# kangxiongbin/HyLight

Measured on AMD Instinct MI355X. Metric: long-read all-vs-all overlaps/sec, higher is better.
Workload: dtype u8/int32

## Files before the change

### hylight_amd/csrc/ava_align.hip

```cpp
#include <algorithm>
#include <memory>
#include <type_traits>

#include "ava_internal.h"
#include "dev_prims.h"
#include "wave_ops.h"

namespace hlmi {

namespace {
constexpr int WG = 256;
constexpr int WAVES = WG / 64;
constexpr int SEQ_T_MAX = EXT_MAX + BAND_W;
constexpr int NR_SHORT = 128;
constexpr int WIDE_SHORT = 128;
inline dim3 grid1(size_t n) { return grid_for(n, WG); }

struct Task {
    uint32_t piece;
    uint16_t kind;
    uint16_t narrow;
    uint64_t qa, ta;
    int16_t m, n;
    int16_t dlo;
    int16_t trim;
};
constexpr uint16_t TASK_REV = 4;
constexpr uint16_t TASK_ONE = 8;
struct TaskOut {
    int32_t score;
    int32_t bi, bj;
    uint32_t runs_off, n_runs;
    uint32_t pad;
// ... 148 lines not shown
    return off;
}

__device__ __forceinline__ uint32_t load_codes4(const uint8_t *base, long long idx, long long total) {
    if (idx >= 0 && idx + 4 <= total) {
        uint32_t v;
        __builtin_memcpy(&v, base + idx, 4);
        return v;
    }
    uint32_t v = 0;
    for (int k = 0; k < 4; ++k) v |= (uint32_t)(idx + k >= 0 && idx + k < total ? base[idx + k] : 4) << (8 * k);
    return v;
}
__device__ __forceinline__ uint32_t comp_codes4(uint32_t x) {
    const uint32_t n = x & 0x04040404u;
    return (x ^ 0x03030303u) & ~((n >> 1) | (n >> 2));
}
__device__ __forceinline__ uint32_t load_window4(const uint8_t *codes, long long total, long long a0, bool down, bool comp, int x) {
    uint32_t v = down ? __builtin_bswap32(load_codes4(codes, a0 - x - 3, total)) : load_codes4(codes, a0 + x, total);
    if (comp) v = comp_codes4(v);
    return v;
}

__device__ __forceinline__ uint32_t load_window4p(const uint8_t *codes, long long a0, bool down, bool comp, int x) {
    uint32_t v;
    __builtin_memcpy(&v, codes + (down ? a0 - x - 3 : a0 + x), 4);
    if (down) v = __builtin_bswap32(v);
    if (comp) v = comp_codes4(v);
    return v;
}


enum { ST_BASES = 0, ST_BASES_SQUARE, ST_BASES_NARROW, ST_BASES_WIDE, ST_FAST, ST_DP, ST_DP_ROWS, ST_NARROW_SMALL, ST_WIDE_ONE, ST_STUB_EXT, ST_EXT_CERT, ST_EXT_DP_ROW, ST_EXT_DP_K, ST_LONG, ST_BASES_LONG, ST_PACKED, N_ALIGN_STATS };
constexpr int NR_SMALL = 64;
constexpr uint8_t CLS_LONG = 5;
constexpr uint8_t CLS_LONG32 = 7;
constexpr uint8_t CLS_UNGAPPED = 6;

__device__ __forceinline__ uint64_t load_codes8(const uint8_t *base, long long idx, long long total) {
    if (idx >= 0 && idx + 8 <= total) {
        uint64_t v;
        __builtin_memcpy(&v, base + idx, 8);
        return v;
    }
    uint64_t v = 0;
    for (int k = 0; k < 8; ++k) v |= (uint64_t)(idx + k >= 0 && idx + k < total ? base[idx + k] : 4) << (8 * k);
    return v;
}
__device__ __forceinline__ uint64_t load_window8(const uint8_t *codes, long long total, long long a0, bool down, bool comp, int x) {
    uint64_t v = down ? __builtin_bswap64(load_codes8(codes, a0 - x - 7, total)) : load_codes8(codes, a0 + x, total);
    if (comp) {
        const uint64_t n = v & 0x0404040404040404ull;
        v = (v ^ 0x0303030303030303ull) & ~((n >> 1) | (n >> 2));
    }
    return v;
}

__device__ __forceinline__ uint64_t load_window8p(const uint8_t *codes, long long a0, bool down, bool comp, int x) {
    uint64_t v;
    __builtin_memcpy(&v, codes + (down ? a0 - x - 7 : a0 + x), 8);
    if (down) v = __builtin_bswap64(v);
    if (comp) {
        const uint64_t n = v & 0x0404040404040404ull;
        v = (v ^ 0x0303030303030303ull) & ~((n >> 1) | (n >> 2));
    }
    return v;
// ... 19 lines not shown
        x = (x | x >> 1) & 0x33333333u;
        x = (x | x >> 2) & 0x0f0f0f0fu;
        x = (x | x >> 4) & 0x00ff00ffu;
        return (x | x >> 8) & 0xffffu;
    };
    return even((uint32_t)d) | even((uint32_t)(d >> 32)) << 16;
}
__device__ __forceinline__ uint32_t squeeze8(uint64_t f) {
    return (((uint32_t)f * 0x10204080u) >> 28) | (((uint32_t)(f >> 32) * 0x10204080u) >> 28) << 4;
}
__device__ __forceinline__ uint32_t ne_bits8(uint64_t q, uint64_t t) {
    const uint64_t d = q ^ t;
    return squeeze8((d | d >> 1 | d >> 2) & 0x0101010101010101ull);
}
__device__ __forceinline__ uint32_t amb_bits8(uint64_t q, uint64_t t) { return squeeze8((q | t) >> 2 & 0x0101010101010101ull); }
__device__ __forceinline__ bool range_flagged(const uint32_t *nflag, long long lo, long long hi) {
    const uint32_t g0 = (uint32_t)((lo + (long long)DevReads::PAD) >> 5), g1 = (uint32_t)((hi + (long long)DevReads::PAD) >> 5);
    uint32_t any = 0;
    for (uint32_t w = g0 >> 5; w <= g1 >> 5; ++w) {
        uint32_t keep = ~0u;
        if (w == g0 >> 5) keep &= ~0u << (g0 & 31);
        if (w == g1 >> 5) keep &= ~0u >> (31 - (g1 & 31));
        any |= nflag[w] & keep;
    }
    return any != 0;
}
__device__ __forceinline__ bool window_flagged(const uint32_t *nflag, long long a0, bool down, int len) {
    return down ? range_flagged(nflag, a0 - (len - 1), a0) : range_flagged(nflag, a0, a0 + (len - 1));
}

template <int PASS>
__global__ __launch_bounds__(WG) __attribute__((amdgpu_waves_per_eu(PASS == 1 ? 4 : 5))) void classify_kernel(AlignArgs a, uint8_t *cls, unsigned long long *stats) {
    __shared__ unsigned long long s_stat[WAVES][N_ALIGN_STATS];
    constexpr int CMP_WORDS = PASS == 1 ? 64 * (BLOCK_MAX / 32) : 1;
    __shared__ uint32_t s_mm[WAVES][CMP_WORDS], s_up[WAVES][CMP_WORDS], s_dn[WAVES][CMP_WORDS];
    __shared__ uint64_t s_qa[WAVES][PASS == 1 ? 64 : 1], s_ta[WAVES][PASS == 1 ? 64 : 1];
    __shared__ uint32_t s_geo[WAVES][PASS == 1 ? 64 : 1], s_amb[WAVES][2];
    const int lane = threadIdx.x & 63;
    const size_t tid = blockIdx.x * (size_t)blockDim.x + threadIdx.x;
    const size_t n_thr = (size_t)gridDim.x * blockDim.x;
    uint32_t chunk_off = 0, chunk_left = 0;
    uint32_t st[N_ALIGN_STATS] = {};
    const size_t n_units = PASS == 1 ? a.n_tasks : (size_t)*a.defer_count;
    const size_t rounds = (n_units + n_thr - 1) / n_thr;
    TaskRef ref_n{0, 0};
    uint32_t ti_n = 0;
    if (PASS == 1) { if (tid < n_units) ref_n = a.geom.ref[tid]; }
    else if (tid < n_units) ti_n = a.defer_list[tid];
    for (size_t r = 0; r < rounds; ++r) {
        const size_t u = r * n_thr + tid;
        bool live = u < n_units;
        const size_t ti = PASS == 1 || !live ? u : (size_t)ti_n;
        TaskRef ref = ref_n;
        if (PASS == 2 && live) ref = a.geom.ref[ti];
        {
            const size_t un = u + n_thr;
            if (PASS == 1) { if (un < n_units) ref_n = a.geom.ref[un]; }
            else if (un < n_units) ti_n = a.defer_list[un];
        }
        Task tk{};
        bool held = false;
        bool bare = false;
        if (live) {
            const uint32_t pc = ref.pk & 0x3fffffffu, kind = ref.pk >> 30;
            const PieceGeom pg = a.geom.pg[pc];
            held = PASS == 1 && kind != 0 && pg.stub_cand != 0;
            bare = a.cls_bare != nullptr && pg.stub_cand != 0;
            const FixPt f0 = a.geom.fps[ref.fp];
            FixPt f1{0, 0};
            if (kind == 0) f1 = a.geom.fps[ref.fp + 1];
            tk = build_task(pg, pc, kind, f0, f1, a.ext_max);
        }
        const int m = tk.m, n = tk.n;
        uint8_t c = 2;
        bool try_fast = false;
        if (live) {
            if (m <= 0 || n <= 0 || held) c = 0;
            else if ((tk.kind & 3) == 0) {
                if (m > BLOCK_MAX || n > BLOCK_MAX)
                    c = (n > m ? n - m : m - n) <= HALF_DELTA ? CLS_LONG32 : CLS_LONG;
                else { c = tk.narrow ? (m <= NR_SHORT ? 1 : 3) : 2; try_fast = (m == n); }
            } else if ((m < n - tk.dlo ? m : n - tk.dlo) > EXT_MAX) { c = CLS_LONG32; tk.dlo = (int16_t)(-(HALF_W / 2 - 1)); }
            else if (a.ext_all_long) c = CLS_LONG;
            if (c == 2 && (m < n - tk.dlo ? m : n - tk.dlo) <= WIDE_SHORT) c = 4;
        }
        if (PASS == 1 && live) {
            const bool defer = c != 0 && a.kmax >= 0 && ((tk.kind & 3) != 0 || (m != n && c != CLS_LONG && c != CLS_LONG32));
            a.defer_flag[ti] = defer ? 1 : 0;
            if (defer) { live = false; try_fast = false; }
        }
        int k = 0, mpos[3] = {0, 0, 0}, last_x = -1;
        bool ambig = false, shift_ok = false;
        if constexpr (PASS == 1) {
            const int wv = threadIdx.x >> 6;
            bool flagged = false;
            if (try_fast && a.qpacked)
                flagged = window_flagged(a.qnflag, (long long)tk.qa, (tk.kind & TASK_REV) != 0, m) || window_flagged(a.tnflag, (long long)tk.ta, false, m);
            const bool use_packed = a.qpacked != nullptr && __ballot(flagged) == 0;
            uint32_t *mm = s_mm[wv], *mup = s_up[wv], *mdn = s_dn[wv];
            const uint32_t nch = try_fast ? (uint32_t)(m + 31) >> 5 : 0u;
            const uint32_t incl = wave_prefix_sum_incl_dpp(nch), tot = (uint32_t)__builtin_amdgcn_readlane((int)incl, 63);
            const uint32_t st0 = incl - nch;
            if (lane < 2) s_amb[wv][lane] = 0;
            s_qa[wv][lane] = tk.qa; s_ta[wv][lane] = tk.ta;
            auto compare = [&](auto packed_form) {
                constexpr bool PK = decltype(packed_form)::value;
                constexpr int PB = PK ? 32 : 8, PW = 32 / PB;
                constexpr uint32_t FIRST = PK ? 3u : 0xffu;
                using piece_t = std::conditional_t<PK, uint32_t, uint8_t>;
                piece_t *own = (piece_t *)mm, *pm = (piece_t *)mm, *pup = (piece_t *)mup, *pdn = (piece_t *)mdn;
                const uint32_t ptot = tot * PW, pst0 = st0 * PW;
                auto window = [&](bool query, int o, bool rv, int x) {
                    if constexpr (PK) return query ? load_window32p(a.qpacked, (long long)s_qa[wv][o], rv, rv, x) : load_window32p(a.tpacked, (long long)s_ta[wv][o], false, false, x);
                    else return query ? load_window8p(a.qcodes, (long long)s_qa[wv][o], rv, rv, x) : load_window8p(a.tcodes, (long long)s_ta[wv][o], false, false, x);
                };
                for (uint32_t c = (uint32_t)lane; c < ptot; c += 64) own[c] = 0;
                s_geo[wv][lane] = pst0 | (uint32_t)m << 16 | ((tk.kind & TASK_REV) ? 0x80000000u : 0u);
                __builtin_amdgcn_s_waitcnt(0xc07f);
                __builtin_amdgcn_wave_barrier();
                if (nch) own[pst0] = (piece_t)lane;
                __builtin_amdgcn_s_waitcnt(0xc07f);
                __builtin_amdgcn_wave_barrier();
// ... 312 lines not shown
        if (bare) nr = 0;
        uint32_t wave_total;
        const uint32_t mine = wave_excl_sum_u32(nr, lane, wave_total);
        uint32_t base = 0;
        bool ok = true;
        if (wave_total) {
            if (lane == 0) base = pool_take(a, wave_total, chunk_off, chunk_left, ok);
            base = (uint32_t)__shfl((int)base, 0, 64);
            ok = __shfl((int)ok, 0, 64) != 0;
        }
        if (fast) {
            if (ok) for (uint32_t q = 0; q < nr; ++q) a.runs[base + mine + q] = runs[q];
            const bool ext = (tk.kind & 3) != 0;
            const int L = ext_take >= 0 ? ext_take : (m < n ? m : n);
            a.out[ti] = TaskOut{fast_score, ext ? L : m, ext ? L : n, base + mine, ok ? nr : 0, (nr ? end_codes(runs[0], runs[nr - 1]) : 0u) | ext_flag};
        } else if (live && c == 0) {
            a.out[ti] = TaskOut{0, 0, 0, 0, 0, 0};
        }
        int m_dp = m;
        if (live && !fast && (c == 1 || c == 3) && a.kmax >= 0 && last_x >= 0 && a.trim_ok && !a.ungapped) {
            const int mn = m < n ? m : n;
            int T = mn - 1 - last_x;
            T = T < mn - 1 ? T : mn - 1;
            if (T > 0) {
                tk.m = (int16_t)(m - T); tk.n = (int16_t)(n - T); tk.trim = (int16_t)T;
                m_dp = m - T;
                c = m_dp <= NR_SHORT ? 1 : 3;
            }
        }
        if (live) {
            if (a.ungapped && c != 0) c = CLS_UNGAPPED;
            cls[ti] = bare ? 0 : c;
            if (a.cls_bare) a.cls_bare[ti] = bare ? c : 0;
            if (c != 0) a.tasks[ti] = tk;
            if (held) ++st[ST_STUB_EXT];
            else if (m > 0 && n > 0) {
                const uint32_t bases = (uint32_t)(m + n);
                st[ST_BASES] += bases;
                if ((tk.kind & 3) == 0 && m == n) st[ST_BASES_SQUARE] += bases;
                if (c == 0) ++st[ST_FAST];
                else {
                    ++st[ST_DP];
                    if (c == CLS_LONG || c == CLS_LONG32) { ++st[ST_LONG]; st[ST_BASES_LONG] += bases; st[ST_DP_ROWS] += (uint32_t)(m < n - tk.dlo ? m : n - tk.dlo); }
                    else if (c == 2 || c == 4) { st[ST_BASES_WIDE] += bases; st[ST_DP_ROWS] += (uint32_t)(m < n - tk.dlo ? m : n - tk.dlo); }
                    else { st[ST_BASES_NARROW] += bases; st[ST_DP_ROWS] += (uint32_t)m_dp; if (c == 1 && m_dp < NR_SMALL && !bare) ++st[ST_NARROW_SMALL]; }
                }
            }
        }
    }
#pragma unroll
    for (int k = 0; k < N_ALIGN_STATS; ++k) {
        unsigned long long v = st[k];
#pragma unroll
        for (int o = 32; o > 0; o >>= 1) v += __shfl_xor(v, o, 64);
        if (lane == 0) s_stat[threadIdx.x >> 6][k] = v;
    }
    __syncthreads();
    if (threadIdx.x < N_ALIGN_STATS) {
        unsigned long long v = 0;
        for (int w = 0; w < WAVES; ++w) v += s_stat[w][threadIdx.x];
        if (v) atomicAdd(&stats[threadIdx.x], v);
    }
}

__global__ void task_rows_key_kernel(const Task *tasks, const uint32_t *list, size_t n, uint32_t *key) {
    size_t i = blockIdx.x * (size_t)blockDim.x + threadIdx.x;
    if (i < n) key[i] = (uint32_t)tasks[list[i]].m >> 2;
}


__global__ void task_rows_desc_key_kernel(const Task *tasks, const uint32_t *list, size_t n, uint32_t *key) {
    size_t i = blockIdx.x * (size_t)blockDim.x + threadIdx.x;
    if (i >= n) return;
    const Task &t = tasks[list[i]];
    const int rows = (int)t.m < (int)t.n - (int)t.dlo ? (int)t.m : (int)t.n - (int)t.dlo;
    key[i] = 0xffffu - (uint32_t)(rows < 0 ? 0 : rows);
}

constexpr int DP_BIAS = 1 << 24;
constexpr int NT_PAD = 16;
constexpr int NT_EXTRA = NT_PAD + NARROW_DELTA + NARROW_W + 7;
enum { PL_DIAG = 0, PL_EGEF, PL_EEXT, PL_FEXT, PL_NE, N_PLANES };

__device__ __forceinline__ uint32_t shift_in(uint32_t acc, bool bit) {
#if defined(__HIP_DEVICE_COMPILE__)
    const unsigned long long m = __ballot(bit);
    unsigned long long co;
    asm("v_addc_co_u32 %0, %1, %2, %2, %3" : "=v"(acc), "=s"(co) : "v"(acc), "s"(m));
#endif
    return acc;
}

struct NarrowWalk {
    const uint32_t *pl;
    int chunks;
// ... 1586 lines not shown
    const size_t n_waves = ((size_t)gridDim.x * blockDim.x) >> 6;
    for (size_t i = wave; i < n; i += n_waves) {
        const Piece p = pieces[i];
        const uint32_t to = off[i];
        for (uint32_t k = (uint32_t)lane; k < p.n_fp; k += 64) dst[to + k] = src[p.fp_off + k];
        if (lane == 0) pieces[i].fp_off = fp_base + to;
    }
}
}

struct PieceSpan { struct { const Piece *p; } pieces; size_t n_pieces, n_fp; struct { const FixPt *p; } fps; };
static void align_span(const AvaInput &in, const hlmi_ava_opts &o, const uint32_t *d_qlen, const uint32_t *d_tlen,
                       const PieceSpan &ch, AlignOut &out) {
    out = AlignOut();
    const size_t P = ch.n_pieces;
    if (!P) return;
    DBuf<uint32_t> tcnt(P), toff(P);
    hipLaunchKernelGGL(piece_task_count_kernel, grid1(P), dim3(WG), 0, stream(), ch.pieces.p, P, tcnt.p);
    exclusive_scan_u32(tcnt.p, toff.p, P);
    const size_t NT = ch.n_fp + P;
    DBuf<Task> tasks(NT);
    if (P >= (1u << 30)) fail(HLMI_EINVAL, "more than 2^30 alignment pieces in one batch");
    DBuf<TaskRef> task_ref(NT);
    DBuf<PieceGeom> pgeom(P);
    if (NT <= 17 * P)
        hipLaunchKernelGGL(task_ref_lane_kernel, grid1(P), dim3(WG), 0, stream(), ch.pieces.p, toff.p, P, d_qlen, d_tlen, in.Q->off.p, in.T->off.p,
                           ch.fps.p, o.stub_oh, ext_rows(o), task_ref.p, pgeom.p);
    else
    hipLaunchKernelGGL(task_ref_kernel, dim3((unsigned)std::min<size_t>(cdiv(P, (size_t)WAVES), 256 * 32)), dim3(WG), 0, stream(),
                       ch.pieces.p, toff.p, P, d_qlen, d_tlen, in.Q->off.p, in.T->off.p, ch.fps.p, o.stub_oh, ext_rows(o), task_ref.p, pgeom.p);
    HIP_CHECK(hipGetLastError());
    DBuf<TaskOut> tout(NT);
    DBuf<uint32_t> counters(2);
    DBuf<unsigned long long> astats(N_ALIGN_STATS);
    constexpr size_t MAX_BLOCKS = 256 * 16;
    const size_t open_chunks = MAX_BLOCKS * (4 * WAVES * RUN_CHUNK + 2 * 4 * WAVES * RUN_CHUNK_SMALL) +
                               (size_t)3 * 256 * 32 * 8 * PK_WAVES * RUN_CHUNK_SMALL;
    size_t run_share = std::max<size_t>(NT * 12, 1 << 16);
    DBuf<uint32_t> runs;
    AsmArgs as{};
    as.pieces = ch.pieces.p; as.fps = ch.fps.p; as.task_off = toff.p; as.tout = tout.p; as.n_pieces = P;
    as.min_dp_score = o.min_dp_score; as.end_bonus = o.end_bonus;
    as.qlen = d_qlen; as.tlen = d_tlen; as.rank_q = in.d_rank_q; as.rank_t = in.d_rank_t; as.chunk_of_t = in.d_chunk_of_t;
    as.pg = pgeom.p; as.stub_score = o.min_dp_score + std::max(0, o.end_bonus);
    as.stage_cap = (uint32_t)ASM_STAGE;
    if (const char *e = hook("HLMI_ASM_STAGE_CAP")) as.stage_cap = (uint32_t)std::min(ASM_STAGE, std::max(0, atoi(e)));
    DBuf<uint32_t> nops(P);
    DBuf<uint8_t> valid(P), late(o.stub_oh >= 0 ? P : 0);
    DBuf<uint32_t> late_idx(o.stub_oh >= 0 ? P : 0);
    size_t n_late = 0;
    const unsigned nba = (unsigned)std::min<size_t>(cdiv(P, (size_t)WAVES), 256 * 32);
    const bool small_pieces = NT <= 17 * P && !hook("HLMI_ASM_WAVE");
    const int worst = std::max(std::max(o.match, o.mismatch), std::max(o.ambi, o.gap_open + o.gap_ext));
    const bool packed = worst > 0 && (long long)worst * (BLOCK_MAX + NARROW_W + 2) <= 4000 && o.match >= 0 && o.mismatch >= 0 &&
                        o.ambi >= 0 && o.gap_open >= 0 && o.gap_ext >= 0 && !hook("HLMI_NARROW_UNPACKED");
    const bool bare = o.stub_oh >= 0 && packed && !hook("HLMI_STUB_FULL_ROWS");
    as.bare = bare ? 1 : 0;
    if (long_rows_cap(o) > 32000) fail(HLMI_EINVAL, "max_gap %d: alignment tasks are limited to 32 000 rows", o.max_gap);
    bool ext_all_long = false;
    if (o.zdrop > 0) {
        const int D = std::max(std::max(o.mismatch, o.ambi), o.gap_open + o.gap_ext);
        const int rows_down = D > 0 ? (o.zdrop + D - 1) / D : EXT_MAX;
        ext_all_long = (long long)o.match * (EXT_MAX - rows_down) + std::max(o.end_bonus, 0) > o.zdrop;
    }
    const uint32_t long_chunks_cap = (uint32_t)(long_rows_cap(o) + 31) / 32, long_runs_cap = (uint32_t)(2 * long_rows_cap(o) + 64);
    constexpr unsigned LONG_BLOCKS_MAX = 256 * 8;
    struct LongLaunch { DBuf<uint32_t> list, planes, runs, ctl; };
    std::vector<std::unique_ptr<LongLaunch>> long_launches;
    struct LongReady { AlignArgs al; LongArgs la; unsigned nb; bool half, tb; const char *timer; };
    std::vector<LongReady> long_ready;
    hipEvent_t long_done = nullptr;
    bool long_pending = false, long_on_side = false;
    struct SideGuard {
        ~SideGuard() { if (hipStream_t s = side_stream_if_created()) (void)hipStreamSynchronize(s); }
    } side_guard;
    auto join_long = [&]() {
        if (!long_pending) return;
        if (long_on_side) {
            if (!long_done) HIP_CHECK(hipEventCreateWithFlags(&long_done, hipEventDisableTiming));
            HIP_CHECK(hipEventRecord(long_done, side_stream()));
            HIP_CHECK(hipStreamWaitEvent(stream(), long_done, 0));
            long_on_side = false;
        }
        long_pending = false;
    };
    DBuf<uint8_t> long_flag;
    DBuf<uint32_t> long_list, long_n(1);
    size_t n_long_tb = 0, n_long_bare = 0;
    double long_rows_run = 0;
    static const char *const LB_NAMES[] = {"align_narrow_small", "align_narrow", "align_narrow_long", "align_wide", "align_wide_short",
                                           "align_long", "align_score_narrow", "align_score_narrow_long", "align_score_wide",
                                           "align_score_wide_short", "align_score_long", "align_ungapped", "align_long32",
                                           "align_score_long32"};
    constexpr int N_LB = 14;
    DBuf<unsigned long long> lb_bases(N_LB + 2);
    std::vector<double> lb_n(N_LB, 0.0);
    lb_bases.zero();
    auto note_list = [&](const char *timer, const Task *tk, const uint32_t *lst, size_t n) {
        if (!n) return;
        int slot = 0;
        while (slot < N_LB && strcmp(LB_NAMES[slot], timer) != 0) ++slot;
        if (slot == N_LB) return;
        lb_n[slot] += (double)n;
        (void)tk; (void)lst;
    };
    for (int attempt = 0;; ++attempt) {
        const size_t cap_runs = run_share + open_chunks;
        if (cap_runs >= (1ull << 32)) fail(HLMI_ENOMEM, "CIGAR run pool exceeds 4G entries");
        runs.alloc(cap_runs);
        counters.zero();
        lb_bases.zero();
        std::fill(lb_n.begin(), lb_n.end(), 0.0);
        AlignArgs aa{};
        aa.tasks = tasks.p; aa.n_tasks = NT;
        aa.geom = TaskGeom{task_ref.p, pgeom.p, ch.fps.p};
        aa.qcodes = in.Q->codes(); aa.tcodes = in.T->codes();
        aa.q_total = (long long)in.Q->total; aa.t_total = (long long)in.T->total;
        if (!hook("HLMI_CLASSIFY_BYTES")) {
            if (!in.Q->packed_store.p || !in.T->packed_store.p) fail(HLMI_ESTATE, "alignment of a read set without its 2-bit copy (DevReads::pack)");
            aa.qpacked = in.Q->packed(); aa.tpacked = in.T->packed();
            aa.qnflag = in.Q->nflag.p; aa.tnflag = in.T->nflag.p;
        }
        aa.end_bonus = o.end_bonus;
        aa.ext_max = ext_rows(o);
        aa.ext_all_long = ext_all_long ? 1 : 0;
        aa.ungapped = o.bandwidth == 0 ? 1 : 0;
        aa.match = o.match; aa.mismatch = o.mismatch; aa.go = o.gap_open; aa.ge = o.gap_ext; aa.ambi = o.ambi;
// ... 4 lines not shown
            const int den = o.match + o.mismatch, num = o.match + 2 * (o.gap_open + o.gap_ext);
            aa.kmax = den > 0 && num > 0 ? std::min(3, (num - 1) / den) : 0;
            if (o.match <= 0 || o.gap_open < 0 || o.gap_ext <= 0) aa.kmax = -1;
            const int k = aa.kmax + 1, U = den, T = num;
            aa.kgap1 = aa.kmax >= 0 && U < o.gap_open + 2 * o.gap_ext + o.match && !hook("HLMI_NO_GAP1_CERT") ? 1 : 0;
            {
                auto c = [&](int L) { int v = o.gap_open + o.gap_ext * L; if (o.gap_open2 > 0) v = std::min(v, o.gap_open2 + o.gap_ext2 * L); return v; };
                aa.kgap2 = aa.kgap1 && U < o.match + c(2) && 2 * U < o.match + 2 * c(1) && 2 * U < 2 * o.match + c(2) + c(3) - c(1) &&
                           c(2) == o.gap_open + 2 * o.gap_ext && c(1) == o.gap_open + o.gap_ext && !hook("HLMI_NO_GAP2_CERT") ? 1 : 0;
            }
            aa.kshift = aa.kmax >= 0 && k <= 3 && k * U > T && k * U < T + o.match + std::min(2 * o.gap_ext, o.gap_open + o.gap_ext) &&
                        !hook("HLMI_NO_SHIFT_CERT") ? 1 : 0;
        }
        aa.trim_ok = hook("HLMI_NO_SUFFIX_TRIM") ? 0 : 1;
        aa.one_ok = hook("HLMI_NO_ONE_PIECE_CERT") ? 0 : 1;
        {
            const int U = o.match + o.mismatch;
            int G = o.gap_open + o.gap_ext;
            if (aa.go2 > 0) G = std::min(G, aa.go2 + aa.ge2);
            const bool sane = aa.kmax >= 0 && o.match > 0 && o.mismatch >= 0 && !hook("HLMI_NO_EXT_CERT");
            aa.kext_plain = sane && G >= U && U < 2 * G + o.match ? 1 : 0;
            aa.kext_bonus = 0;
            for (int k = 1; k <= 2; ++k)
                if (sane && o.end_bonus > 0 && k * U < G && k * U < o.end_bonus + o.match && k * U < 2 * G + o.match) aa.kext_bonus = k;
        }
        aa.out = tout.p; aa.runs = runs.p; aa.cap_runs = (uint32_t)cap_runs; aa.counters = counters.p;
        as.runs = runs.p;
        aa.run_buf_cap = 0xffffffffu;
        if (const char *e = hook("HLMI_RUN_BUF_CAP")) aa.run_buf_cap = (uint32_t)std::max(0, atoi(e));
        DBuf<uint8_t> cls(NT), f1(NT), cls_bare(bare ? NT : 0);
        DBuf<uint32_t> list1(NT), list2(NT), list3(NT), list4(NT);
        DBuf<uint32_t> list_n(4);
        aa.cls_bare = bare ? cls_bare.p : nullptr;
        auto class_list = [&](const uint8_t *cls_arr, uint8_t v) -> size_t {
            if (long_flag.n < NT) { long_flag.alloc(NT); long_list.alloc(NT); }
            hipLaunchKernelGGL(class_flag_kernel, grid1(NT), dim3(WG), 0, stream(), cls_arr, NT, v, long_flag.p);
            select_flagged_indices_async(long_flag.p, long_list.p, NT, long_n.p);
            return (size_t)long_n.download(1)[0];
        };
        auto run_ungapped = [&](const uint8_t *cls_arr, bool tb) -> size_t {
            if (!aa.ungapped) return 0;
            const size_t nl = class_list(cls_arr, CLS_UNGAPPED);
            if (!nl) return 0;
            aa.list = long_list.p; aa.n_list = nl;
            note_list("align_ungapped", tasks.p, long_list.p, nl);
            KTimer kt("align_ungapped");
            const unsigned nb = (unsigned)std::min<size_t>(cdiv(nl, (size_t)WG), MAX_BLOCKS);
            if (tb) hipLaunchKernelGGL(align_ungapped_kernel<true>, dim3(nb), dim3(WG), 0, stream(), aa, o.zdrop);
            else hipLaunchKernelGGL(align_ungapped_kernel<false>, dim3(nb), dim3(WG), 0, stream(), aa, o.zdrop);
            HIP_CHECK(hipGetLastError());
            return nl;
        };
        auto run_long_class = [&](const uint8_t *cls_arr, bool tb, uint8_t cv) -> size_t {
            const bool half = cv == CLS_LONG32;
            const char *timer = half ? (tb ? "align_long32" : "align_score_long32") : (tb ? "align_long" : "align_score_long");
            const size_t nl = class_list(cls_arr, cv);
            if (!nl) return 0;
            note_list(timer, tasks.p, long_list.p, nl);
            hipLaunchKernelGGL(list_ext_kernel, dim3((unsigned)std::min<size_t>(cdiv(nl, (size_t)WG), 1024)), dim3(WG), 0, stream(), tasks.p,
                               long_list.p, nl, lb_bases.p + N_LB);
            long_launches.emplace_back(new LongLaunch());
            LongLaunch &L = *long_launches.back();
            {
                DBuf<uint32_t> key(nl);
                hipLaunchKernelGGL(task_rows_desc_key_kernel, grid1(nl), dim3(WG), 0, stream(), tasks.p, long_list.p, nl, key.p);
                L.list.alloc(nl);
                HIP_CHECK(hipMemcpyAsync(L.list.p, long_list.p, nl * 4, hipMemcpyDeviceToDevice, stream()));
                sort_pairs_u32_u32(key, L.list, nl, 0, 16);
            }
            const size_t units = half ? (nl + 1) / 2 : nl;
            const unsigned nb = (unsigned)std::min<size_t>((units + WAVES - 1) / WAVES, LONG_BLOCKS_MAX);
// ... 28 lines not shown
                } else {
                    if (r.tb) { if (two) go(align_long_kernel<true, true>); else go(align_long_kernel<false, true>); }
                    else { if (two) go(align_long_kernel<true, false>); else go(align_long_kernel<false, false>); }
                }
            }
            HIP_CHECK(hipGetLastError());
            long_ready.clear();
            long_pending = true;
        };
        auto run_long = [&](const uint8_t *cls_arr, bool tb) -> size_t {
            if (aa.ungapped) return run_ungapped(cls_arr, tb);
            const size_t n32 = run_long_class(cls_arr, tb, CLS_LONG32);
            return n32 + run_long_class(cls_arr, tb, CLS_LONG);
        };
        auto check_long = [&]() {
            for (auto &L : long_launches) {
                if (!L->ctl.n) continue;
                const std::vector<uint32_t> c = L->ctl.download(4);
                if (c[1]) fail(HLMI_EINVAL, "an alignment task exceeds the scratch area of align_long_kernel");
                long_rows_run += (double)((unsigned long long)c[3] << 32 | c[2]);
                L->ctl.release(); L->planes.release(); L->runs.release(); L->list.release();
            }
        };
        size_t n_bare_tasks = 0;
        auto run_bare_long = [&]() {
            if (!bare) return;
            const size_t nl = run_long(cls_bare.p, false);
            n_bare_tasks += nl; n_long_bare += nl;
        };
        auto run_bare = [&](bool with_long) {
            if (!bare) return;
            if (with_long) { run_bare_long(); launch_long_ready(); }
            select_classes4_async(cls_bare.p, NT, list1.p, list2.p, list3.p, list4.p, list_n.p);
            const std::vector<uint32_t> hb = list_n.download(4);
            n_bare_tasks += (size_t)hb[0] + hb[1] + hb[2] + hb[3];
            for (int which = 0; which < 2; ++which) {
                DBuf<uint32_t> &lst = which ? list3 : list1;
                const size_t nl = which ? hb[2] : hb[0];
                if (nl < 8) continue;
                DBuf<uint32_t> key(nl);
                hipLaunchKernelGGL(task_rows_key_kernel, grid1(nl), dim3(WG), 0, stream(), tasks.p, lst.p, nl, key.p);
                sort_pairs_u32_u32(key, lst, nl, 0, 7);
            }
            auto pk_grid = [](size_t n) { return dim3((unsigned)std::max<size_t>(1, std::min<size_t>(((n + 7) / 8 + PK_WAVES - 1) / PK_WAVES, 256 * 32))); };
            auto w_grid = [](size_t n) { return dim3((unsigned)std::max<size_t>(1, std::min<size_t>((n + WAVES - 1) / WAVES, 256 * 16))); };
            if (hb[0]) {
                note_list("align_score_narrow", tasks.p, list1.p, hb[0]);
                KTimer kt("align_score_narrow");
                aa.list = list1.p; aa.n_list = hb[0];
                hipLaunchKernelGGL((align_narrow_pk_kernel<NR_SHORT, false>), pk_grid(hb[0]), dim3(64 * PK_WAVES), 0, stream(), aa);
            }
            if (hb[2]) {
                note_list("align_score_narrow_long", tasks.p, list3.p, hb[2]);
                KTimer kt("align_score_narrow_long");
                aa.list = list3.p; aa.n_list = hb[2];
                hipLaunchKernelGGL((align_narrow_pk_kernel<BLOCK_MAX, false>), pk_grid(hb[2]), dim3(64 * PK_WAVES), 0, stream(), aa);
            }
            if (hb[1]) {
                note_list("align_score_wide", tasks.p, list2.p, hb[1]);
                KTimer kt("align_score_wide");
                aa.list = list2.p; aa.n_list = hb[1];
                hipLaunchKernelGGL((align_kernel<EXT_MAX, false>), w_grid(hb[1]), dim3(WG), 0, stream(), aa);
            }
            if (hb[3]) {
                note_list("align_score_wide_short", tasks.p, list4.p, hb[3]);
                KTimer kt("align_score_wide_short");
                aa.list = list4.p; aa.n_list = hb[3];
                hipLaunchKernelGGL((align_kernel<WIDE_SHORT, false>), w_grid(hb[3]), dim3(WG), 0, stream(), aa);
            }
        };
        {
            KTimer kt("align_classify");
            const unsigned nbc = (unsigned)std::min<size_t>(cdiv(NT, (size_t)WG), MAX_BLOCKS);
            astats.zero();
            aa.defer_flag = f1.p;
            aa.defer_list = list1.p; aa.defer_count = list_n.p;
            hipLaunchKernelGGL(classify_kernel<1>, dim3(nbc ? nbc : 1), dim3(WG), 0, stream(), aa, cls.p, astats.p);
            select_flagged_indices_async(f1.p, list1.p, NT, list_n.p);
            const unsigned nb2 = std::max(1u, nbc / 4);
            hipLaunchKernelGGL(classify_kernel<2>, dim3(nb2), dim3(WG), 0, stream(), aa, cls.p, astats.p);
        }
        HIP_CHECK(hipGetLastError());
        hipLaunchKernelGGL(class_bases_kernel, dim3((unsigned)std::min<size_t>(cdiv(NT, (size_t)WG), 2048)), dim3(WG), 0, stream(), cls.p,
                           bare ? cls_bare.p : nullptr, tasks.p, NT, lb_bases.p);
        select_classes4_async(cls.p, NT, list1.p, list2.p, list3.p, list4.p, list_n.p);
        const std::vector<uint32_t> hn = list_n.download(4);
        const size_t n1 = hn[0], n2 = hn[1], n3 = hn[2], n4 = hn[3];
        for (int which = 0; which < 2; ++which) {
            DBuf<uint32_t> &lst = which ? list3 : list1;
            const size_t nl = which ? n3 : n1;
            if (nl < 8) continue;
            DBuf<uint32_t> key(nl);
            hipLaunchKernelGGL(task_rows_key_kernel, grid1(nl), dim3(WG), 0, stream(), tasks.p, lst.p, nl, key.p);
            sort_pairs_u32_u32(key, lst, nl, 0, 7);
        }
        unsigned long long long_seen = astats.download(N_ALIGN_STATS)[ST_LONG];
        if (long_seen || aa.ungapped) {
            run_bare_long();
            n_long_tb += run_long(cls.p, true);
            launch_long_ready();
        }
        if (n1 && packed) {
            size_t n_small = 0;
            if (n1 >= 8) n_small = std::min<size_t>(n1, (size_t)astats.download(N_ALIGN_STATS)[ST_NARROW_SMALL]);
            if (n_small) {
                note_list("align_narrow_small", tasks.p, list1.p, n_small);
                KTimer kt("align_narrow_small");
                aa.list = list1.p; aa.n_list = n_small;
                const unsigned nb = (unsigned)std::min<size_t>(((n_small + 7) / 8 + PK_WAVES - 1) / PK_WAVES, 256 * 32);
                hipLaunchKernelGGL(align_narrow_pk_kernel<NR_SMALL>, dim3(nb ? nb : 1), dim3(64 * PK_WAVES), 0, stream(), aa);
            }
            if (n1 > n_small) {
                note_list("align_narrow", tasks.p, list1.p + n_small, n1 - n_small);
                KTimer kt("align_narrow");
                aa.list = list1.p + n_small; aa.n_list = n1 - n_small;
                const unsigned nb = (unsigned)std::min<size_t>(((aa.n_list + 7) / 8 + PK_WAVES - 1) / PK_WAVES, 256 * 32);
                hipLaunchKernelGGL(align_narrow_pk_kernel<NR_SHORT>, dim3(nb ? nb : 1), dim3(64 * PK_WAVES), 0, stream(), aa);
            }
        } else if (n1) {
            note_list("align_narrow", tasks.p, list1.p, n1);
            KTimer kt("align_narrow");
            aa.list = list1.p; aa.n_list = n1;
            const unsigned nb = (unsigned)std::min<size_t>(((n1 + 3) / 4 + WAVES - 1) / WAVES, 256 * 16);
            hipLaunchKernelGGL(align_narrow_kernel<NR_SHORT>, dim3(nb ? nb : 1), dim3(WG), 0, stream(), aa);
        }
        if (n3 && packed && !hook("HLMI_NARROW_LONG_UNPACKED")) {
            note_list("align_narrow_long", tasks.p, list3.p, n3);
            KTimer kt("align_narrow_long");
            aa.list = list3.p; aa.n_list = n3;
            const unsigned nb = (unsigned)std::min<size_t>(((n3 + 7) / 8 + PK_WAVES - 1) / PK_WAVES, 256 * 32);
            hipLaunchKernelGGL(align_narrow_pk_kernel<BLOCK_MAX>, dim3(nb ? nb : 1), dim3(64 * PK_WAVES), 0, stream(), aa);
        } else if (n3) {
            note_list("align_narrow_long", tasks.p, list3.p, n3);
            KTimer kt("align_narrow_long");
            aa.list = list3.p; aa.n_list = n3;
            const unsigned nb = (unsigned)std::min<size_t>(((n3 + 3) / 4 + WAVES - 1) / WAVES, 256 * 16);
            hipLaunchKernelGGL(align_narrow_kernel<BLOCK_MAX>, dim3(nb ? nb : 1), dim3(WG), 0, stream(), aa);
// ... 11 lines not shown
                KTimer kt("align_wide_short");
                aa.list = list4.p; aa.n_list = n_short;
                const unsigned nb = (unsigned)std::min<size_t>((n_short + WAVES - 1) / WAVES, 256 * 16);
                hipLaunchKernelGGL(align_kernel<WIDE_SHORT>, dim3(nb ? nb : 1), dim3(WG), 0, stream(), aa);
            }
        };
        run_wide(n2, n4);
        run_bare(false);
        size_t n_wide_late = 0;
        if (o.stub_oh >= 0) {
            as.plist = nullptr; as.n_pieces = P; as.late = late.p;
            join_long();
            {
                KTimer kt("assemble_count");
                if (small_pieces) hipLaunchKernelGGL(assemble_lane_kernel<false>, grid1(as.n_pieces), dim3(WG), 0, stream(), as, nops.p, valid.p,
                                                     nullptr, nullptr, nullptr, nullptr, nullptr);
                else
                hipLaunchKernelGGL(assemble_kernel<false>, dim3(nba), dim3(WG), 0, stream(), as, nops.p, valid.p, nullptr, nullptr,
                                   nullptr, nullptr, nullptr);
            }
            as.late = nullptr;
            n_late = select_flagged_indices(late.p, late_idx.p, P);
            if (n_late) {
                hipLaunchKernelGGL(late_tasks_kernel, grid1(n_late), dim3(WG), 0, stream(), late_idx.p, n_late, ch.pieces.p, toff.p,
                                   list1.p, list_n.p);
                HIP_CHECK(hipMemsetAsync(cls.p, 0, NT, stream()));
                if (bare) HIP_CHECK(hipMemsetAsync(cls_bare.p, 0, NT, stream()));
                {
                    KTimer kt("align_classify");
                    aa.defer_list = list1.p; aa.defer_count = list_n.p;
                    const unsigned nb2 = (unsigned)std::min<size_t>(cdiv(2 * n_late, (size_t)WG), MAX_BLOCKS);
                    hipLaunchKernelGGL(classify_kernel<2>, dim3(nb2 ? nb2 : 1), dim3(WG), 0, stream(), aa, cls.p, astats.p);
                }
                hipLaunchKernelGGL(class_bases_kernel, dim3((unsigned)std::min<size_t>(cdiv(NT, (size_t)WG), 2048)), dim3(WG), 0, stream(), cls.p,
                                   bare ? cls_bare.p : nullptr, tasks.p, NT, lb_bases.p);
                if (bare) {
                    const size_t before = n_bare_tasks;
                    const bool more_long = astats.download(N_ALIGN_STATS)[ST_LONG] > long_seen || aa.ungapped;
                    run_bare(more_long);
                    n_wide_late = n_bare_tasks - before;
                } else {
                    select_classes4_async(cls.p, NT, list1.p, list2.p, list3.p, list4.p, list_n.p);
                    const std::vector<uint32_t> hl = list_n.download(4);
                    run_wide(hl[1], hl[3]);
                    const bool more_long = astats.download(N_ALIGN_STATS)[ST_LONG] > long_seen || aa.ungapped;
                    const size_t nl = more_long ? run_long(cls.p, true) : 0;
                    launch_long_ready();
                    n_long_tb += nl;
                    n_wide_late = (size_t)hl[1] + hl[3] + nl;
                }
                as.plist = late_idx.p; as.n_pieces = n_late;
                const unsigned nbl = (unsigned)std::min<size_t>(cdiv(n_late, (size_t)WAVES), 256 * 32);
                join_long();
                {
                    KTimer kt("assemble_count");
                    if (small_pieces) hipLaunchKernelGGL(assemble_lane_kernel<false>, grid1(as.n_pieces), dim3(WG), 0, stream(), as, nops.p, valid.p,
                                                         nullptr, nullptr, nullptr, nullptr, nullptr);
                    else
                    hipLaunchKernelGGL(assemble_kernel<false>, dim3(nbl), dim3(WG), 0, stream(), as, nops.p, valid.p, nullptr, nullptr,
                                       nullptr, nullptr, nullptr);
                }
                as.plist = nullptr; as.n_pieces = P;
            }
        }
        if (attempt == 0) {
            stat_add("align_tasks_narrow", (double)(n1 + n3)); stat_add("align_tasks_wide", (double)(n2 + n4 + (bare ? 0 : n_wide_late)));
            stat_add("align_tasks_score_only", (double)n_bare_tasks);
            stat_add("align_tasks_long", (double)n_long_tb); stat_add("align_tasks_long_score_only", (double)n_long_bare);
        }
        HIP_CHECK(hipGetLastError());
        join_long();
        std::vector<uint32_t> hc = counters.download(2);
        check_long();
        if (!hc[1]) break;
        if (attempt >= 3) fail(HLMI_ENOMEM, "CIGAR run pool overflow");
        run_share *= 4;
    }
    stat_add("align_tasks", (double)NT);
    {
        std::vector<unsigned long long> h = astats.download(N_ALIGN_STATS);
        stat_add("align_tasks_fast", (double)h[ST_FAST]);
        stat_add("align_tasks_packed", (double)h[ST_PACKED]);
        stat_add("align_tasks_dp", (double)h[ST_DP]);
        stat_add("align_dp_rows", (double)h[ST_DP_ROWS]);
        stat_add("align_dp_bases", (double)h[ST_BASES]);
        stat_add("align_bases_classify", (double)h[ST_BASES_SQUARE]);
        stat_add("align_bases_narrow", (double)h[ST_BASES_NARROW]);
        stat_add("align_bases_wide", (double)h[ST_BASES_WIDE]);
        stat_add("align_bases_long", (double)h[ST_BASES_LONG]);
        const std::vector<unsigned long long> lb = lb_bases.download(N_LB + 2);
        stat_add("align_long_rows_run", long_rows_run);
        stat_add("align_long_ext", (double)lb[N_LB]);
        stat_add("align_long_ext_rows", (double)lb[N_LB + 1]);
        for (int k = 0; k < N_LB; ++k)
            if (lb_n[k] > 0) {
                stat_add(std::string("align_n.") + LB_NAMES[k], lb_n[k]);
                stat_add(std::string("align_bases.") + LB_NAMES[k], (double)lb[k]);
            }
        stat_add("align_tasks_wide_one_piece", (double)h[ST_WIDE_ONE]);
        stat_add("align_ext_certified", (double)h[ST_EXT_CERT]);
        stat_add("align_ext_dp_bonus_row_elsewhere", (double)h[ST_EXT_DP_ROW]);
        stat_add("align_ext_dp_substitutions", (double)h[ST_EXT_DP_K]);
        stat_add("align_ext_held", (double)h[ST_STUB_EXT]);
        stat_add("align_ext_late", (double)(2 * n_late));
    }
    if (o.stub_oh < 0) {
        KTimer kt("assemble_count");
        if (small_pieces) hipLaunchKernelGGL(assemble_lane_kernel<false>, grid1(as.n_pieces), dim3(WG), 0, stream(), as, nops.p, valid.p,
                                             nullptr, nullptr, nullptr, nullptr, nullptr);
        else
        hipLaunchKernelGGL(assemble_kernel<false>, dim3(nba), dim3(WG), 0, stream(), as, nops.p, valid.p, nullptr, nullptr,
                           nullptr, nullptr, nullptr);
    }
    HIP_CHECK(hipGetLastError());
    DBuf<uint64_t> ooff(P);
    exclusive_scan_u32_to_u64(nops.p, ooff.p, P);
    const size_t n_ops = (size_t)(download_one(ooff.p + (P - 1)) + download_one(nops.p + (P - 1)));
    DBuf<uint32_t> vidx(P);
    const size_t R = select_flagged_indices(valid.p, vidx.p, P);
    if (!R) return;
    out.ops.alloc(n_ops ? n_ops : 1);
    DBuf<PafRec> recs(P);
    DBuf<uint64_t> hi(P), lo(P);
// ... 105 lines not shown
```

### hylight_amd/csrc/runtime.cpp

```cpp
#include <mutex>

#include "common.h"
#include <sched.h>

#include <iterator>

namespace hlmi {

namespace {
thread_local std::string g_last_error;
bool g_ready = false;
int g_device = 0;
int g_threads = 0;
std::map<std::string, double> g_stats;
std::mutex g_mu;
std::mutex g_stat_mu;

struct KRec { std::string name; hipEvent_t a, b; hipStream_t s; };
struct Lane {
    hipStream_t stream = nullptr, side = nullptr;
    std::vector<KRec> krecs;
    void *pinned = nullptr;
};
Lane g_lanes[MAX_LANES];
// ... 119 lines not shown

int lane_count() {
    int n = 2;
    if (const char *e = hook("HLMI_LANES")) n = atoi(e);
    return std::max(1, std::min(n, MAX_LANES));
}
LaneScope::LaneScope(int id) : prev(t_lane) {
    if (id < 0 || id >= MAX_LANES) fail(HLMI_EINVAL, "lane %d out of range", id);
    t_lane = id;
    HIP_CHECK(hipSetDevice(g_device));
    if (!lane().stream) HIP_CHECK(hipStreamCreateWithFlags(&lane().stream, hipStreamNonBlocking));
}
LaneScope::~LaneScope() {
    lane_drain();
    try { ktimer_flush(); } catch (...) {}
    t_lane = prev;
}

namespace {
const char *const HOOK_NAMES[] = {
    "HLMI_ALIGN_SPAN_TASKS",
    "HLMI_ANCHOR_BATCH_M",
    "HLMI_ANCHOR_PAIRS",
    "HLMI_ANCHOR_SPLIT",
    "HLMI_ASM_STAGE_CAP",
    "HLMI_ASM_WAVE",
    "HLMI_CHAIN_DP16_CHECK",
    "HLMI_CHAIN_NO_DP16",
    "HLMI_CHAIN_NO_SMALL",
    "HLMI_SEED_GROUP", "HLMI_TEXT_GPU", "HLMI_TEXT_HOST", "HLMI_GRAPH_WINDOW_MB", "HLMI_LANES", "HLMI_SET_ASIDE_CUTS", "HLMI_SEED_NO_GUESS",
    "HLMI_CHAIN_PROF",
    "HLMI_CHAIN_UNPACKED",
    "HLMI_CLASSIFY_BYTES",
    "HLMI_GROUP_HIST",
    "HLMI_HOST_TIMERS",
    "HLMI_LONG_SIDE_STREAM",
    "HLMI_NARROW_LONG_UNPACKED",
    "HLMI_NARROW_UNPACKED",
    "HLMI_NO_EXT_CERT",
    "HLMI_POLISH_ROWS_GRID",
    "HLMI_NO_GAP1_CERT",
    "HLMI_NO_GAP2_CERT",
    "HLMI_NO_ONE_PIECE_CERT",
    "HLMI_NO_RANK_WORD",
    "HLMI_NO_SHIFT_CERT",
    "HLMI_NO_STUB",
    "HLMI_NO_SUFFIX_TRIM",
    "HLMI_QCAP_MIN",
    "HLMI_RUN_BUF_CAP",
    "HLMI_SKETCH_PART_MBASES",
    "HLMI_SNP_SORT",
    "HLMI_STUB_FULL_ROWS",
    "HLMI_SUBRUN_MAX_MANCHORS",
    "HLMI_SUBRUN_MAX_OUT_MB",
    "HLMI_SUBRUN_MBASES"};
std::unordered_map<std::string, std::string> g_hooks;
}
void hooks_refresh() {
    g_hooks.clear();
    for (const char *n : HOOK_NAMES)
        if (const char *v = getenv(n)) g_hooks[n] = v;
}
const char *hook(const char *name) {
    bool known = false;
    for (const char *n : HOOK_NAMES) known = known || strcmp(n, name) == 0;
    if (!known) fail(HLMI_EINVAL, "hook %s is not in the table of runtime.cpp", name);
// ... 154 lines not shown
```

Baseline: 3659.

## Count class sizes and bases inside classify kernel to drop host syncs

The classify kernel now accumulates, in shared memory, per-class task counts, bare counts, deferred counts and per-slot base sums, then flushes them to the stats buffer. The host reads these counts in a single download instead of several list_n/astats downloads, and class_list skips empty classes without syncing. The separate class_bases_kernel launch runs only behind a debug hook that cross-checks the sums. Extra shared atomics are added to the classifier, and a host wait timer is recorded as a stat.

```diff
diff --git a/hylight_amd/csrc/ava_align.hip b/hylight_amd/csrc/ava_align.hip
--- a/hylight_amd/csrc/ava_align.hip
+++ b/hylight_amd/csrc/ava_align.hip
@@ -1,4 +1,5 @@
 #include <algorithm>
+#include <chrono>
 #include <memory>
 #include <type_traits>
 
@@ -213,6 +214,7 @@
 
 
 enum { ST_BASES = 0, ST_BASES_SQUARE, ST_BASES_NARROW, ST_BASES_WIDE, ST_FAST, ST_DP, ST_DP_ROWS, ST_NARROW_SMALL, ST_WIDE_ONE, ST_STUB_EXT, ST_EXT_CERT, ST_EXT_DP_ROW, ST_EXT_DP_K, ST_LONG, ST_BASES_LONG, ST_PACKED, N_ALIGN_STATS };
+enum { CS_BASES = 0, N_LB_SLOTS = 14, CS_N = CS_BASES + N_LB_SLOTS, N_CLS = 7, CS_N_BARE = CS_N + N_CLS, CS_DEFER = CS_N_BARE + N_CLS, N_CLASS_STATS };
 constexpr int NR_SMALL = 64;
 constexpr uint8_t CLS_LONG = 5;
 constexpr uint8_t CLS_LONG32 = 7;
@@ -298,6 +300,9 @@
 template <int PASS>
 __global__ __launch_bounds__(WG) __attribute__((amdgpu_waves_per_eu(PASS == 1 ? 4 : 5))) void classify_kernel(AlignArgs a, uint8_t *cls, unsigned long long *stats) {
     __shared__ unsigned long long s_stat[WAVES][N_ALIGN_STATS];
+    __shared__ unsigned long long s_cls[N_CLASS_STATS];
+    if (threadIdx.x < N_CLASS_STATS) s_cls[threadIdx.x] = 0;
+    __syncthreads();
     constexpr int CMP_WORDS = PASS == 1 ? 64 * (BLOCK_MAX / 32) : 1;
     __shared__ uint32_t s_mm[WAVES][CMP_WORDS], s_up[WAVES][CMP_WORDS], s_dn[WAVES][CMP_WORDS];
     __shared__ uint64_t s_qa[WAVES][PASS == 1 ? 64 : 1], s_ta[WAVES][PASS == 1 ? 64 : 1];
@@ -353,7 +358,7 @@
         if (PASS == 1 && live) {
             const bool defer = c != 0 && a.kmax >= 0 && ((tk.kind & 3) != 0 || (m != n && c != CLS_LONG && c != CLS_LONG32));
             a.defer_flag[ti] = defer ? 1 : 0;
-            if (defer) { live = false; try_fast = false; }
+            if (defer) { live = false; try_fast = false; atomicAdd(&s_cls[CS_DEFER], 1ull); }
         }
         int k = 0, mpos[3] = {0, 0, 0}, last_x = -1;
         bool ambig = false, shift_ok = false;
@@ -732,7 +737,15 @@
             if (a.ungapped && c != 0) c = CLS_UNGAPPED;
             cls[ti] = bare ? 0 : c;
             if (a.cls_bare) a.cls_bare[ti] = bare ? c : 0;
-            if (c != 0) a.tasks[ti] = tk;
+            if (c != 0) {
+                a.tasks[ti] = tk;
+                const int rows = tk.m, cols = tk.n;
+                int slot;
+                if (!bare) slot = c == 1 ? (rows < NR_SMALL ? 0 : 1) : c == 3 ? 2 : c == 2 ? 3 : c == 4 ? 4 : c == CLS_LONG ? 5 : c == CLS_LONG32 ? 12 : 11;
+                else slot = c == 1 ? 6 : c == 3 ? 7 : c == 2 ? 8 : c == 4 ? 9 : c == CLS_LONG ? 10 : c == CLS_LONG32 ? 13 : 11;
+                atomicAdd(&s_cls[CS_BASES + slot], (unsigned long long)(rows + cols));
+                atomicAdd(&s_cls[(bare ? CS_N_BARE : CS_N) + c - 1], 1ull);
+            }
             if (held) ++st[ST_STUB_EXT];
             else if (m > 0 && n > 0) {
                 const uint32_t bases = (uint32_t)(m + n);
@@ -761,6 +774,7 @@
         for (int w = 0; w < WAVES; ++w) v += s_stat[w][threadIdx.x];
         if (v) atomicAdd(&stats[threadIdx.x], v);
     }
+    if (threadIdx.x < N_CLASS_STATS && s_cls[threadIdx.x]) atomicAdd(&stats[N_ALIGN_STATS + threadIdx.x], s_cls[threadIdx.x]);
 }
 
 __global__ void task_rows_key_kernel(const Task *tasks, const uint32_t *list, size_t n, uint32_t *key) {
@@ -2413,7 +2427,8 @@
     HIP_CHECK(hipGetLastError());
     DBuf<TaskOut> tout(NT);
     DBuf<uint32_t> counters(2);
-    DBuf<unsigned long long> astats(N_ALIGN_STATS);
+    constexpr size_t N_ASTATS = N_ALIGN_STATS + N_CLASS_STATS;
+    DBuf<unsigned long long> astats(N_ASTATS);
     constexpr size_t MAX_BLOCKS = 256 * 16;
     const size_t open_chunks = MAX_BLOCKS * (4 * WAVES * RUN_CHUNK + 2 * 4 * WAVES * RUN_CHUNK_SMALL) +
                                (size_t)3 * 256 * 32 * 8 * PK_WAVES * RUN_CHUNK_SMALL;
@@ -2465,6 +2480,13 @@
         }
         long_pending = false;
     };
+    double host_wait = 0;
+    auto waited = [&](auto &&fetch) {
+        const auto t0 = std::chrono::steady_clock::now();
+        auto v = fetch();
+        host_wait += std::chrono::duration<double>(std::chrono::steady_clock::now() - t0).count();
+        return v;
+    };
     DBuf<uint8_t> long_flag;
     DBuf<uint32_t> long_list, long_n(1);
     size_t n_long_tb = 0, n_long_bare = 0;
@@ -2474,6 +2496,8 @@
                                            "align_score_wide_short", "align_score_long", "align_ungapped", "align_long32",
                                            "align_score_long32"};
     constexpr int N_LB = 14;
+    static_assert(N_LB == N_LB_SLOTS, "the classifier sums bases per LB_NAMES slot");
+    const bool bases_pass = hook("HLMI_CLASS_BASES_PASS") != nullptr;
     DBuf<unsigned long long> lb_bases(N_LB + 2);
     std::vector<double> lb_n(N_LB, 0.0);
     lb_bases.zero();
@@ -2544,11 +2568,28 @@
         DBuf<uint32_t> list1(NT), list2(NT), list3(NT), list4(NT);
         DBuf<uint32_t> list_n(4);
         aa.cls_bare = bare ? cls_bare.p : nullptr;
+        std::vector<unsigned long long> h_stats(N_ASTATS, 0);
+        size_t cn[N_CLS + 1] = {}, cnb[N_CLS + 1] = {};
+        auto fetch_counts = [&]() {
+            const std::vector<unsigned long long> now = waited([&] { return astats.download(N_ASTATS); });
+            for (int c = 1; c <= N_CLS; ++c) {
+                cn[c] = (size_t)(now[N_ALIGN_STATS + CS_N + c - 1] - h_stats[N_ALIGN_STATS + CS_N + c - 1]);
+                cnb[c] = (size_t)(now[N_ALIGN_STATS + CS_N_BARE + c - 1] - h_stats[N_ALIGN_STATS + CS_N_BARE + c - 1]);
+            }
+            h_stats = now;
+        };
+        auto class_bases_pass = [&]() {
+            if (!bases_pass) return;
+            hipLaunchKernelGGL(class_bases_kernel, dim3((unsigned)std::min<size_t>(cdiv(NT, (size_t)WG), 2048)), dim3(WG), 0, stream(), cls.p,
+                               bare ? cls_bare.p : nullptr, tasks.p, NT, lb_bases.p);
+        };
         auto class_list = [&](const uint8_t *cls_arr, uint8_t v) -> size_t {
+            const size_t nl = (cls_arr == cls.p ? cn : cnb)[v];
+            if (!nl) return 0;
             if (long_flag.n < NT) { long_flag.alloc(NT); long_list.alloc(NT); }
             hipLaunchKernelGGL(class_flag_kernel, grid1(NT), dim3(WG), 0, stream(), cls_arr, NT, v, long_flag.p);
             select_flagged_indices_async(long_flag.p, long_list.p, NT, long_n.p);
-            return (size_t)long_n.download(1)[0];
+            return nl;
         };
         auto run_ungapped = [&](const uint8_t *cls_arr, bool tb) -> size_t {
             if (!aa.ungapped) return 0;
@@ -2643,7 +2684,7 @@
             if (!bare) return;
             if (with_long) { run_bare_long(); launch_long_ready(); }
             select_classes4_async(cls_bare.p, NT, list1.p, list2.p, list3.p, list4.p, list_n.p);
-            const std::vector<uint32_t> hb = list_n.download(4);
+            const size_t hb[4] = {cnb[1], cnb[2], cnb[3], cnb[4]};
             n_bare_tasks += (size_t)hb[0] + hb[1] + hb[2] + hb[3];
             for (int which = 0; which < 2; ++which) {
                 DBuf<uint32_t> &lst = which ? list3 : list1;
@@ -2692,11 +2733,10 @@
             hipLaunchKernelGGL(classify_kernel<2>, dim3(nb2), dim3(WG), 0, stream(), aa, cls.p, astats.p);
         }
         HIP_CHECK(hipGetLastError());
-        hipLaunchKernelGGL(class_bases_kernel, dim3((unsigned)std::min<size_t>(cdiv(NT, (size_t)WG), 2048)), dim3(WG), 0, stream(), cls.p,
-                           bare ? cls_bare.p : nullptr, tasks.p, NT, lb_bases.p);
+        class_bases_pass();
         select_classes4_async(cls.p, NT, list1.p, list2.p, list3.p, list4.p, list_n.p);
-        const std::vector<uint32_t> hn = list_n.download(4);
-        const size_t n1 = hn[0], n2 = hn[1], n3 = hn[2], n4 = hn[3];
+        fetch_counts();
+        const size_t n1 = cn[1], n2 = cn[2], n3 = cn[3], n4 = cn[4];
         for (int which = 0; which < 2; ++which) {
             DBuf<uint32_t> &lst = which ? list3 : list1;
             const size_t nl = which ? n3 : n1;
@@ -2705,7 +2745,7 @@
             hipLaunchKernelGGL(task_rows_key_kernel, grid1(nl), dim3(WG), 0, stream(), tasks.p, lst.p, nl, key.p);
             sort_pairs_u32_u32(key, lst, nl, 0, 7);
         }
-        unsigned long long long_seen = astats.download(N_ALIGN_STATS)[ST_LONG];
+        const unsigned long long long_seen = h_stats[ST_LONG];
         if (long_seen || aa.ungapped) {
             run_bare_long();
             n_long_tb += run_long(cls.p, true);
@@ -2713,7 +2753,7 @@
         }
         if (n1 && packed) {
             size_t n_small = 0;
-            if (n1 >= 8) n_small = std::min<size_t>(n1, (size_t)astats.download(N_ALIGN_STATS)[ST_NARROW_SMALL]);
+            if (n1 >= 8) n_small = std::min<size_t>(n1, (size_t)h_stats[ST_NARROW_SMALL]);
             if (n_small) {
                 note_list("align_narrow_small", tasks.p, list1.p, n_small);
                 KTimer kt("align_narrow_small");
@@ -2791,18 +2831,17 @@
                     const unsigned nb2 = (unsigned)std::min<size_t>(cdiv(2 * n_late, (size_t)WG), MAX_BLOCKS);
                     hipLaunchKernelGGL(classify_kernel<2>, dim3(nb2 ? nb2 : 1), dim3(WG), 0, stream(), aa, cls.p, astats.p);
                 }
-                hipLaunchKernelGGL(class_bases_kernel, dim3((unsigned)std::min<size_t>(cdiv(NT, (size_t)WG), 2048)), dim3(WG), 0, stream(), cls.p,
-                                   bare ? cls_bare.p : nullptr, tasks.p, NT, lb_bases.p);
+                class_bases_pass();
+                if (!bare) select_classes4_async(cls.p, NT, list1.p, list2.p, list3.p, list4.p, list_n.p);
+                fetch_counts();
+                const bool more_long = h_stats[ST_LONG] > long_seen || aa.ungapped;
                 if (bare) {
                     const size_t before = n_bare_tasks;
-                    const bool more_long = astats.download(N_ALIGN_STATS)[ST_LONG] > long_seen || aa.ungapped;
                     run_bare(more_long);
                     n_wide_late = n_bare_tasks - before;
                 } else {
-                    select_classes4_async(cls.p, NT, list1.p, list2.p, list3.p, list4.p, list_n.p);
-                    const std::vector<uint32_t> hl = list_n.download(4);
+                    const size_t hl[4] = {cn[1], cn[2], cn[3], cn[4]};
                     run_wide(hl[1], hl[3]);
-                    const bool more_long = astats.download(N_ALIGN_STATS)[ST_LONG] > long_seen || aa.ungapped;
                     const size_t nl = more_long ? run_long(cls.p, true) : 0;
                     launch_long_ready();
                     n_long_tb += nl;
@@ -2836,8 +2875,9 @@
         run_share *= 4;
     }
     stat_add("align_tasks", (double)NT);
+    stat_add("wall_s.align_host_wait", host_wait);
     {
-        std::vector<unsigned long long> h = astats.download(N_ALIGN_STATS);
+        std::vector<unsigned long long> h = astats.download(N_ASTATS);
         stat_add("align_tasks_fast", (double)h[ST_FAST]);
         stat_add("align_tasks_packed", (double)h[ST_PACKED]);
         stat_add("align_tasks_dp", (double)h[ST_DP]);
@@ -2847,7 +2887,13 @@
         stat_add("align_bases_narrow", (double)h[ST_BASES_NARROW]);
         stat_add("align_bases_wide", (double)h[ST_BASES_WIDE]);
         stat_add("align_bases_long", (double)h[ST_BASES_LONG]);
-        const std::vector<unsigned long long> lb = lb_bases.download(N_LB + 2);
+        std::vector<unsigned long long> lb = lb_bases.download(N_LB + 2);
+        for (int k = 0; k < N_LB; ++k) {
+            const unsigned long long counted = h[N_ALIGN_STATS + CS_BASES + k];
+            if (bases_pass && lb[k] != counted)
+                fail(HLMI_EINVAL, "HLMI_CLASS_BASES_PASS: %s: the classifier counted %llu bases, class_bases_kernel %llu", LB_NAMES[k], counted, lb[k]);
+            lb[k] = counted;
+        }
         stat_add("align_long_rows_run", long_rows_run);
         stat_add("align_long_ext", (double)lb[N_LB]);
         stat_add("align_long_ext_rows", (double)lb[N_LB + 1]);
diff --git a/hylight_amd/csrc/runtime.cpp b/hylight_amd/csrc/runtime.cpp
--- a/hylight_amd/csrc/runtime.cpp
+++ b/hylight_amd/csrc/runtime.cpp
@@ -175,6 +175,7 @@
     "HLMI_CHAIN_PROF",
     "HLMI_CHAIN_UNPACKED",
     "HLMI_CLASSIFY_BYTES",
+    "HLMI_CLASS_BASES_PASS",
     "HLMI_GROUP_HIST",
     "HLMI_HOST_TIMERS",
     "HLMI_LONG_SIDE_STREAM",
```

Result: no change. 3669 (median of 2 runs) (+0.3%).
